# aproposorg/sydr

Hardware: AMD Instinct MI355X
Metric: IQ Msamples/s through 32-ch E/P/L correlators @25 MHz fs (higher is better)
Workload: dtype f64

## Files before the change

### sydr_amd/csrc/correlator_chip.h

```cpp
#pragma once

#include "correlator.h"

#pragma clang fp contract(off)

namespace sdr {

constexpr int kChipMax = 26;
constexpr double kChipMinCodeStep = 1.0 / 25.9;
constexpr double kChipMaxCodeStep = 1.0 / 15.5;
constexpr int kChipRawDwords = 13;
constexpr int kChipRotSlots = 2 * kChipMax + 2;
template <int NT>
constexpr int chip_strip_slots() { return 2 * NT + 1; }

__host__ __device__ __forceinline__ int chip_first_above(double thr, double shift, double inv_step, bool& near) {
    const double u = (thr - shift) * inv_step;
    const double fl = floor(u);
    const double fr = u - fl;
    near = near || fr < kNearInteger || fr > 1.0 - kNearInteger;
    return (int)fl + 1;
}
__host__ __device__ __forceinline__ int chip_first_above_exact(int c, double thr, double step, double shift) {
    auto above = [&](int i) {
        double y = (double)i * step;
        y = y + shift;
        return y > thr;
    };
    if (c >= 1 && above(c - 1)) return (c >= 2 && above(c - 2)) ? c - 2 : c - 1;
    if (c < 0) c = 0;
    if (above(c)) return c;
    return above(c + 1) ? c + 1 : c + 2;
}

template <int B, int E, class F>
__device__ __forceinline__ void static_for(F&& f) {
    if constexpr (B < E) {
        f(std::integral_constant<int, B>{});
        static_for<B + 1, E>(f);
    }
}

__device__ __forceinline__ int wave_min_i32(int x) {
#pragma unroll
    for (int off = 1; off < 64; off <<= 1) {
        const int o = __shfl_xor(x, off, 64);
        x = o < x ? o : x;
    }
    return __builtin_amdgcn_readfirstlane(x);
}

#ifndef SDR_BIASED_CVT
#define SDR_BIASED_CVT 1
#endif
constexpr double kCvtBias = 4224.0;
typedef uint32_t sdr_u32x2 __attribute__((ext_vector_type(2)));
__device__ __forceinline__ double biased_sample(sdr_u32x2& pair, uint32_t w_flipped, uint32_t selector, uint32_t hi_const) {
    pair.y = __builtin_amdgcn_perm(w_flipped, hi_const, selector);
    return __builtin_bit_cast(double, pair);
}
constexpr uint32_t cvt_selector(int byte) { return 0x03020000u | ((uint32_t)(4 + byte) << 8) | 0x0Cu; }

template <int NT>
struct ChipGeom {
    int64_t Tfx, Ufx;
    uint64_t delta[NT];
    int q0, F;
    int head_end, tail_start;
    int m[NT], J[NT];
    int bad;
};

template <int NT, int KM, int KS, int KI>
__host__ __device__ __forceinline__ void chip_geometry(int n, const double* shift, const double* step, const double* inv_step,
                                                       ChipGeom<NT>& g) {
    constexpr int A = NT / 2;
    const double two32 = 4294967296.0;
    g.q0 = (int)ceil(shift[A]);
    double y_last = (double)(n - 1) * step[A];
    y_last = y_last + shift[A];
    const int q_last = (int)ceil(y_last);
    g.F = q_last - g.q0 - 1;
    g.head_end = n, g.tail_start = n;
    if (g.F > 0) {
        bool nr = false;
        g.head_end = chip_first_above_exact(chip_first_above((double)g.q0, shift[A], inv_step[A], nr), (double)g.q0, step[A], shift[A]);
        g.tail_start = chip_first_above_exact(chip_first_above((double)(q_last - 1), shift[A], inv_step[A], nr),
                                              (double)(q_last - 1), step[A], shift[A]);
    }
    g.Tfx = (int64_t)rint(inv_step[A] * two32);
    g.Ufx = (int64_t)floor(-shift[A] * inv_step[A] * two32);
    const int M = (int)(g.Tfx >> 32);
    bool bad = M < 1 || M + 1 > kChipMax || g.F > 16384 || (KM != 0 && M != KM);
#pragma unroll
    for (int t = 0; t < NT; ++t) {
        g.m[t] = M, g.J[t] = 0, g.delta[t] = 0;
        if (t == A) continue;
        const int64_t Ut = (int64_t)floor(-shift[t] * inv_step[t] * two32);
        int j = (int)ceil(shift[t] - shift[A]) - 1;
        int64_t d = (Ut - g.Ufx) + (int64_t)(1 + j) * g.Tfx;
        if (d < 0) {
            d += g.Tfx;
            ++j;
        } else if (d >= g.Tfx) {
            d -= g.Tfx;
            --j;
        }
        bad = bad || d < 0 || d >= g.Tfx;
        g.J[t] = j;
        g.delta[t] = (uint64_t)d;
        g.m[t] = (int)(d >> 32);
        bad = bad || (KS != 0 && (g.m[t] != KS || j != (t < A ? -1 : 0)));
        bad = bad || (KI != 0 && !((j == (t - A) * KI - 1 && g.m[t] == 0) || (j == (t - A) * KI && g.m[t] >= M)));
    }
    g.bad = bad ? 1 : 0;
}

constexpr int kStaticHalf = 13;
constexpr int chip_half(int KM, int KS, int KI) { return KI != 0 ? (KM + 2) / 2 : KS + 1; }
struct ChipRot {
    double urc[kStaticHalf + 1], urs[kStaticHalf + 1];
    double rd0c, rd0s, rd1c, rd1s;
    double biasc[3], biass[3];
};
__host__ __device__ inline void chip_rotations(double dphi, int Dmin, ChipRot& r, int half = kStaticHalf, int cmin = kStaticHalf - 2) {
    double cs[16], sn[16];
    for (int k = 0; k < 16; ++k) sincos_reduced(-(double)k * dphi, &sn[k], &cs[k]);
    for (int k = 1; k <= half; ++k) r.urc[k] = cs[k], r.urs[k] = sn[k];
    r.urc[0] = 1.0, r.urs[0] = 0.0;
    sincos_reduced(-(double)Dmin * dphi, &r.rd0s, &r.rd0c);
    sincos_reduced(-(double)(Dmin + 1) * dphi, &r.rd1s, &r.rd1c);
    for (int st = 1; st < 16; st <<= 1)
        for (int l = 15; l >= st; --l) cs[l] += cs[l - st], sn[l] += sn[l - st];
    for (int i = 0; i < 3; ++i) {
        const int l = cmin + i - 1;
        const double re = cs[l] - sn[l], im = cs[l] + sn[l];
        r.biasc[i] = re * 4224.0, r.biass[i] = im * 4224.0;
    }
}

template <int NT>
struct ChipSetup {
    double dphi;
    double shift[NT], step[NT], inv_step[NT];
    int64_t base;
    ChipGeom<NT> g;
    ChipRot r;
};

template <int NT, int KM, int KS, int KI>
__host__ __device__ inline void chip_setup(int n, int64_t start_sample, int64_t capacity, double carrier_hz, double rem_code,
                                           double code_step, const double* spacing, double fs, int stride, ChipSetup<NT>& S) {
    S = ChipSetup<NT>{};
    S.dphi = carrier_step(carrier_hz, fs);
    const double nd = (double)n;
    for (int t = 0; t < NT; ++t) {
        const double shift = rem_code + spacing[t];
        double stop = code_step * nd;
        stop = stop + shift;
        const double delta = stop - shift;
        S.shift[t] = shift;
        S.step[t] = delta / nd;
        S.inv_step[t] = 1.0 / S.step[t];
    }
    const int64_t base = start_sample % capacity;
    const bool applies = code_step >= kChipMinCodeStep && code_step <= kChipMaxCodeStep && base + n + 32 <= capacity;
    S.base = applies ? base : -1;
    if (applies) {
        chip_geometry<NT, KM, KS, KI>(n, S.shift, S.step, S.inv_step, S.g);
        chip_rotations(S.dphi, (int)(((int64_t)stride * S.g.Tfx) >> 32), S.r, chip_half(KM, KS, KI), KM - chip_half(KM, KS, KI));
    }
}

template <int NT>
struct ChipBlock {
    uint32_t raw[kChipRawDwords];
    int S;
    int dn;
    int ds[NT];
};

template <int NT, bool SINGLE_WAVE, int KM = 0, int KS = 0, int KI = 0>
__device__ __forceinline__ bool correlate_epoch_chip(const void* __restrict__ ring, const void* __restrict__ ring_flipped, int64_t capacity,
                                                     const EpochParams& ep, double dphi, const EpochConsts<NT>& K,
                                                     const ChipGeom<NT>& G, int64_t base, const ChipRot* R,
                                                     const uint32_t* lut, double2* strip_lds, double2* rot, int tid,
                                                     int lane, int stride, int edge_lane, double* accr, double* acci) {
    constexpr int A = NT / 2;
    constexpr int kSlots = chip_strip_slots<NT>();
    const int n = ep.n;
    const double* shift = K.shift;
    const double* step = K.step;
    double2* strip = strip_lds + tid * kSlots;
    const int wlane = threadIdx.x & 63;
#pragma unroll
    for (int t = 0; t < NT; ++t) accr[t] = acci[t] = 0.0;

    const double dphi_u = uniform(dphi), rem_carrier_u = uniform(ep.rem_carrier);
    const int q0 = __builtin_amdgcn_readfirstlane(G.q0);
    const int F = __builtin_amdgcn_readfirstlane(G.F);
    const int head_end = __builtin_amdgcn_readfirstlane(G.head_end);
    const int tail_start = __builtin_amdgcn_readfirstlane(G.tail_start);
    (void)ring_flipped;
    const char* ring_base = static_cast<const char*>(ring) + base * 2;

    static_assert(!(KS != 0 && KI != 0), "either the taps switch inside the block (KS) or with it (KI)");
    constexpr bool kStatic = KM != 0 && (KS != 0 || KI != 0);
    constexpr int kHalf = chip_half(KM, KS, KI);
    double urc[kStatic ? kHalf + 1 : 1], urs[kStatic ? kHalf + 1 : 1];
    double biasc[3] = {0.0, 0.0, 0.0}, biass[3] = {0.0, 0.0, 0.0};
    const double two32 = 4294967296.0;
    int64_t Tfx = G.Tfx;
    int64_t stride_fx = (int64_t)stride * Tfx;
    const int Dmin = (int)(stride_fx >> 32);
    if constexpr (kStatic) asm volatile("" : "+v"(Tfx), "+v"(stride_fx));
    double rd0c = 1.0, rd0s = 0.0, rd1c = 1.0, rd1s = 0.0;
    {
        double sn = 0.0, cs = 0.0;
        if constexpr (kStatic) {
            static_assert(kHalf <= kStaticHalf, "the plan's rotations are laid out for half blocks of up to 13 samples");
#pragma unroll
            for (int k = 1; k <= kHalf; ++k) urc[k] = R->urc[k], urs[k] = R->urs[k];
            rd0c = R->rd0c, rd0s = R->rd0s, rd1c = R->rd1c, rd1s = R->rd1s;
            if constexpr (SDR_BIASED_CVT) {
#pragma unroll
                for (int i = 0; i < 3; ++i) biasc[i] = R->biasc[i], biass[i] = R->biass[i];
            }
        } else {
            if (wlane < kChipMax) {
                sincos_reduced(-(double)wlane * dphi_u, &sn, &cs);
                rot[wlane] = make_double2(cs, sn);
            }
            if constexpr (SDR_BIASED_CVT) {
                double br = (cs - sn) * kCvtBias, bi = (cs + sn) * kCvtBias;
#pragma unroll
                for (int off = 1; off < 32; off <<= 1) {
                    const double o_r = __shfl_up(br, off, 64), o_i = __shfl_up(bi, off, 64);
                    br = wlane >= off ? br + o_r : br;
                    bi = wlane >= off ? bi + o_i : bi;
                }
                double2* const btab = rot + kChipMax;
                if (wlane < kChipMax) btab[wlane + 1] = make_double2(br, bi);
                if (wlane == 0) btab[0] = make_double2(0.0, 0.0);
            }
        }
    }

    bool bad = false;
    const int rounds = F > 0 ? (F + stride - 1) / stride : 0;
    if (rounds > 0) {
        int64_t Ufx = G.Ufx;
        const int M = (int)(G.Tfx >> 32);
        if constexpr (kStatic) asm volatile("" : "+v"(Ufx));
        bad = bad || G.bad != 0;
        int m[NT], J[NT];
        uint64_t delta[NT];
        unsigned evmask = (1u << M) | (2u << M);
#pragma unroll
        for (int t = 0; t < NT; ++t) {
            m[t] = G.m[t], J[t] = G.J[t], delta[t] = G.delta[t];
            if constexpr (kStatic) asm volatile("" : "+v"(m[t]), "+v"(J[t]), "+v"(delta[t]));
            if (t != A) evmask |= (1u << m[t]) | (2u << m[t]);
        }
        const int k_last = M + 1;
        int rank[NT];
#pragma unroll
        for (int t = 0; t < NT; ++t) rank[t] = __builtin_popcount(evmask & ((1u << m[t]) - 1u));
        if constexpr (!kStatic) {
            double sn, cs;
            sincos_reduced(-(double)(Dmin + (wlane & 1)) * dphi_u, &sn, &cs);
            rd0c = lane_value(cs, 0), rd0s = lane_value(sn, 0);
            rd1c = lane_value(cs, 1), rd1s = lane_value(sn, 1);
        }
        asm volatile("" : "+v"(rd0c), "+v"(rd0s), "+v"(rd1c), "+v"(rd1s));
        const uint64_t lane_fx = (uint64_t)((int64_t)lane * Tfx);
        uint64_t u_cur = (uint64_t)(Ufx + (int64_t)q0 * Tfx + (int64_t)two32) + lane_fx;
        const int last_idx = F - 1;

        auto prepare = [&](int round, uint64_t u0, ChipBlock<NT>& b) {
            const int idx = round * stride + lane;
            const bool inside = idx <= last_idx;
            const uint64_t uS = inside ? u0 : (uint64_t)(Ufx + (int64_t)(q0 + last_idx) * Tfx + (int64_t)two32);
            const uint64_t uE = uS + (uint64_t)Tfx;
            int S = (int)(uS >> 32);
            int E = (int)(uE >> 32);
            bool near = (uint32_t)uS + 0x10000u < 0x20000u || (uint32_t)uE + 0x10000u < 0x20000u;
            int split[NT];
#pragma unroll
            for (int t = 0; t < NT; ++t) {
                split[t] = 0;
                if (t == A) continue;
                if constexpr (KI != 0) {
                    split[t] = J[t] == (t - A) * KI ? E - S : 0;
                    continue;
                }
                const uint64_t uT = uS + delta[t];
                near = near || (uint32_t)uT + 0x10000u < 0x20000u;
                split[t] = (int)(uT >> 32) - S;
            }
            if (__builtin_expect(__any(near), 0)) {
                const int q = q0 + 1 + (inside ? idx : last_idx);
                S = chip_first_above_exact(S, (double)(q - 1), step[A], shift[A]);
                E = chip_first_above_exact(E, (double)q, step[A], shift[A]);
#pragma unroll
                for (int t = 0; t < NT; ++t) {
                    if (t == A) continue;
                    const int p0 = q + J[t];
                    const int bt = chip_first_above_exact(S + split[t], (double)p0, step[t], shift[t]);
                    double y = (double)S * step[t];
                    y = y + shift[t];
                    const int at_s = (int)ceil(y);
                    bad = bad || (at_s != p0 && at_s != p0 + 1) || (at_s == p0 + 1 && bt > S);
                    split[t] = bt < S ? 0 : bt - S;
                }
            }
            b.S = S;
            const int nn = E - S;
            b.dn = nn - M;
            bad = bad || (unsigned)b.dn > 1u;
#pragma unroll
            for (int t = 0; t < NT; ++t) {
                b.ds[t] = 0;
                if (t == A) continue;
                const int sp = split[t] > nn ? nn : split[t];
                if constexpr (KI != 0) {
                    bad = bad || !(J[t] == (t - A) * KI ? sp == nn : sp == 0);
                    continue;
                }
                b.ds[t] = sp - m[t];
                bad = bad || (unsigned)b.ds[t] > 1u;
            }
            if constexpr (KS != 0 && NT == 3) bad = bad || b.ds[0] != b.ds[2];
            const char* src = ring_base + (int64_t)S * 2;
            const uint4 w0 = *reinterpret_cast<const uint4*>(src);
            const uint4 w1 = *reinterpret_cast<const uint4*>(src + 16);
            const uint4 w2 = *reinterpret_cast<const uint4*>(src + 32);
            const uint32_t w3 = *reinterpret_cast<const uint32_t*>(src + 48);
            b.raw[0] = w0.x, b.raw[1] = w0.y, b.raw[2] = w0.z, b.raw[3] = w0.w;
            b.raw[4] = w1.x, b.raw[5] = w1.y, b.raw[6] = w1.z, b.raw[7] = w1.w;
            b.raw[8] = w2.x, b.raw[9] = w2.y, b.raw[10] = w2.z, b.raw[11] = w2.w;
            b.raw[12] = w3;
        };

        ChipBlock<NT> blk_a, blk_b;
        prepare(0, u_cur, blk_a);
        double sb, cb;
        sincos_reduced(__builtin_fma(-(double)blk_a.S, dphi_u, rem_carrier_u), &sb, &cb);
        if constexpr (!kStatic) {
            sb = lane <= last_idx ? sb : 0.0;
            cb = lane <= last_idx ? cb : 0.0;
        }
        const int q_lane = q0 + 1 + lane + SDR_LUT_PAD;
        const uint32_t* zero_lq = reinterpret_cast<const uint32_t*>(strip) + 3;
        if constexpr (kStatic) strip[0] = strip[1] = make_double2(0.0, 0.0);

        sdr_u32x2 zI = {0u, 0u}, zQ = {0u, 0u};
        asm volatile("" : "+v"(zI), "+v"(zQ));

        auto process = [&](const ChipBlock<NT>& b, int round, double sbk, double cbk) {
            double pr = 0.0, pi = 0.0;
            double2* wp = strip;
            unsigned evm = evmask;
            int klast = k_last;
            if constexpr (!kStatic) asm volatile("" : "+s"(evm), "+s"(klast));
            constexpr int kAhead = 4;
            double2 rr[kChipMax + kAhead];
            if constexpr (!kStatic) {
#pragma unroll
                for (int k = 0; k < kAhead; ++k) rr[k] = rot[k];
            }
            auto park = [&]() {
                *wp = make_double2(pr, pi);
                ++wp;
                asm volatile("" ::: "memory");
            };
            uint32_t hi_rt = 0x40B00000u;
            uint32_t sel_rt[4] = {cvt_selector(0), cvt_selector(1), cvt_selector(2), cvt_selector(3)};
            if constexpr (!kStatic && SDR_BIASED_CVT) {
                asm volatile("" : "+v"(hi_rt));
                asm volatile("" : "+s"(sel_rt[0]), "+s"(sel_rt[1]), "+s"(sel_rt[2]), "+s"(sel_rt[3]));
            }
            auto sample = [&](auto kc) {
                constexpr int k = decltype(kc)::value;
                double ar, ai;
                if constexpr (SDR_BIASED_CVT) {
                    ar = biased_sample(zI, b.raw[k >> 1], sel_rt[(k & 1) ? 2 : 0], hi_rt);
                    ai = biased_sample(zQ, b.raw[k >> 1], sel_rt[(k & 1) ? 3 : 1], hi_rt);
                } else {
                    const int w = ci8_native((int)b.raw[k >> 1]);
                    ar = (k & 1) ? (double)(int)(int8_t)(w >> 16) : (double)(int)(int8_t)w;
                    ai = (k & 1) ? (double)(w >> 24) : (double)(int)(int8_t)(w >> 8);
                }
                if (k + kAhead < kChipMax) rr[k + kAhead] = rot[k + kAhead];
                const double2 r = rr[k];
                pr = __builtin_fma(-ai, r.y, __builtin_fma(ar, r.x, pr));
                pi = __builtin_fma(ai, r.x, __builtin_fma(ar, r.y, pi));
                if constexpr (SDR_BIASED_CVT) asm volatile("" : "+v"(pr), "+v"(pi), "+v"(zI), "+v"(zQ));
            };
            double capr[3] = {0.0, 0.0, 0.0}, capi[3] = {0.0, 0.0, 0.0};
            if constexpr (kStatic) {
                static_assert(2 * kHalf >= KM + 1 && kHalf < KM, "two halves of at most KS + 1 samples cover the block");
                static_assert(!SDR_BIASED_CVT || (2 * kHalf - KM >= 1 && 2 * kHalf - KM <= 2 && (KS == 0 || KS == kHalf - 1)),
                              "the offset's shares are kept for sums of KM - kHalf, + 1 and + 2 samples: kHalf must be one of the last two");
                uint32_t flipped[kChipRawDwords];
                uint32_t hi_const = 0x40B00000u;
                if constexpr (SDR_BIASED_CVT) {
                    asm volatile("" : "+v"(hi_const));
#pragma unroll
                    for (int i = 0; i < kChipRawDwords; ++i) flipped[i] = b.raw[i];
                }
                static_for<0, KM + 1>([&](auto kc) {
                    constexpr int k = decltype(kc)::value;
                    constexpr int j = k < kHalf ? k : k - kHalf;
                    const int w = ci8_native((int)b.raw[k >> 1]);
                    double ar, ai;
                    if constexpr (SDR_BIASED_CVT) {
                        ar = biased_sample(zI, flipped[k >> 1], cvt_selector((k & 1) ? 2 : 0), hi_const);
                        ai = biased_sample(zQ, flipped[k >> 1], cvt_selector((k & 1) ? 3 : 1), hi_const);
                    } else {
                        ar = (k & 1) ? (double)(int)(int8_t)(w >> 16) : (double)(int)(int8_t)w;
                        ai = (k & 1) ? (double)(w >> 24) : (double)(int)(int8_t)(w >> 8);
                    }
                    if constexpr (KS != 0 && k == KS) capr[0] = pr, capi[0] = pi;
                    if constexpr (k == KM) capr[1] = pr, capi[1] = pi;
                    if constexpr (k == kHalf) capr[2] = pr, capi[2] = pi;
                    if constexpr (j == 0) {
                        pr = ar, pi = ai;
                    } else {
                        pr = __builtin_fma(-ai, urs[j], __builtin_fma(ar, urc[j], pr));
                        pi = __builtin_fma(ai, urc[j], __builtin_fma(ar, urs[j], pi));
                    }
                    if constexpr (SDR_BIASED_CVT) asm volatile("" : "+v"(pr), "+v"(pi), "+v"(zI), "+v"(zQ));
                });
            } else if constexpr (KM != 0) {
                static_for<0, KM>([&](auto kc) {
                    constexpr int k = decltype(kc)::value;
                    if (evm & (1u << k)) park();
                    sample(kc);
                });
                park();
                sample(std::integral_constant<int, KM>{});
                park();
            } else {
#pragma unroll
                for (int k = 0; k <= kChipMax; ++k) {
                    if (evm & (1u << k)) {
                        park();
                        if (k == klast) break;
                    }
                    if (k < kChipMax) {
                        double ar, ai;
                        if constexpr (SDR_BIASED_CVT) {
                            ar = biased_sample(zI, b.raw[k >> 1], sel_rt[(k & 1) ? 2 : 0], hi_rt);
                            ai = biased_sample(zQ, b.raw[k >> 1], sel_rt[(k & 1) ? 3 : 1], hi_rt);
                        } else {
                            const int w = ci8_native((int)b.raw[k >> 1]);
                            ar = (k & 1) ? (double)(int)(int8_t)(w >> 16) : (double)(int)(int8_t)w;
                            ai = (k & 1) ? (double)(w >> 24) : (double)(int)(int8_t)(w >> 8);
                        }
                        if (k + kAhead < kChipMax) rr[k + kAhead] = rot[k + kAhead];
                        const double2 r = rr[k];
                        pr = __builtin_fma(-ai, r.y, __builtin_fma(ar, r.x, pr));
                        pi = __builtin_fma(ai, r.x, __builtin_fma(ar, r.y, pi));
                        if constexpr (SDR_BIASED_CVT) asm volatile("" : "+v"(pr), "+v"(pi), "+v"(zI), "+v"(zQ));
                    }
                }
            }
            double2 ptot;
            if constexpr (kStatic && SDR_BIASED_CVT) {
                constexpr int iFirst = 2 * kHalf - KM;
                pr -= biasc[1], pi -= biass[1];
                capr[1] -= biasc[0], capi[1] -= biass[0];
                capr[2] -= biasc[iFirst], capi[2] -= biass[iFirst];
                if constexpr (KS != 0) capr[0] -= biasc[iFirst - 1], capi[0] -= biass[iFirst - 1];
            }
            if constexpr (kStatic) {
                const double qr = b.dn ? pr : capr[1], qi = b.dn ? pi : capi[1];
                ptot.x = __builtin_fma(-qi, urs[kHalf], __builtin_fma(qr, urc[kHalf], capr[2]));
                ptot.y = __builtin_fma(qi, urc[kHalf], __builtin_fma(qr, urs[kHalf], capi[2]));
            } else {
                ptot = strip[rank[A] + b.dn];
                if constexpr (SDR_BIASED_CVT) {
                    const double2 bb = (rot + kChipMax)[M + b.dn];
                    ptot.x -= bb.x, ptot.y -= bb.y;
                }
            }
            const int first = round * stride;
            const uint32_t* lq;
            if constexpr (kStatic)
                lq = first + lane <= last_idx ? lut + q_lane + first : zero_lq;
            else
                lq = lut + q_lane + (first + lane <= last_idx ? first : last_idx - lane);
            if constexpr (KI != 0) {
                const double xr = __builtin_fma(-sbk, ptot.y, cbk * ptot.x);
                const double xi = __builtin_fma(sbk, ptot.x, cbk * ptot.y);
#pragma unroll
                for (int t = 0; t < NT; ++t) {
                    const double c = __hiloint2double((int)lq[(t - A) * KI], 0);
                    accr[t] = __builtin_fma(c, xr, accr[t]);
                    acci[t] = __builtin_fma(c, xi, acci[t]);
                }
                return;
            }
#pragma unroll
            for (int t = 0; t < NT; ++t) {
                double gr, gi;
                if (t == A) {
                    const double c = __hiloint2double((int)lq[0], 0);
                    gr = c * ptot.x;
                    gi = c * ptot.y;
                } else {
                    double2 ps;
                    if constexpr (kStatic)
                        ps = b.ds[NT == 3 ? 0 : t] ? make_double2(capr[2], capi[2]) : make_double2(capr[0], capi[0]);
                    else {
                        ps = strip[rank[t] + b.ds[t]];
                        if constexpr (SDR_BIASED_CVT) {
                            const double2 bb = (rot + kChipMax)[m[t] + b.ds[t]];
                            ps.x -= bb.x, ps.y -= bb.y;
                        }
                    }
                    const int jt = kStatic ? (t < A ? -1 : 0) : J[t];
                    const double ca = __hiloint2double((int)lq[jt], 0);
                    const double cbn = __hiloint2double((int)lq[jt + 1], 0);
                    const double diff = ca - cbn;
                    gr = __builtin_fma(diff, ps.x, cbn * ptot.x);
                    gi = __builtin_fma(diff, ps.y, cbn * ptot.y);
                }
                accr[t] = __builtin_fma(-sbk, gi, __builtin_fma(cbk, gr, accr[t]));
                acci[t] = __builtin_fma(sbk, gr, __builtin_fma(cbk, gi, acci[t]));
            }
        };

        auto wave_has_work = [&](int round) { return SINGLE_WAVE || round * stride + (lane - wlane) <= last_idx; };
        auto advance = [&](const ChipBlock<NT>& from, const ChipBlock<NT>& to, int to_round) {
            const unsigned dd = (unsigned)(to.S - from.S - Dmin);
            const bool alive = to_round * stride + lane <= last_idx;
            bad = bad || (alive && dd > 1u);
            const double rc_ = dd ? rd1c : rd0c, rs_ = dd ? rd1s : rd0s;
            const double cbn = __builtin_fma(cb, rc_, -sb * rs_);
            const double sbn = __builtin_fma(sb, rc_, cb * rs_);
            if constexpr (kStatic) {
                cb = cbn, sb = sbn;
            } else {
                cb = alive ? cbn : 0.0;
                sb = alive ? sbn : 0.0;
            }
        };

        for (int it = 0; it < rounds / 2; ++it) {
            const double sb0 = sb, cb0 = cb;
            u_cur += (uint64_t)stride_fx;
            prepare(2 * it + 1, u_cur, blk_b);
            advance(blk_a, blk_b, 2 * it + 1);
            if (wave_has_work(2 * it)) process(blk_a, 2 * it, sb0, cb0);
            const double sb1 = sb, cb1 = cb;
            if (2 * it + 2 < rounds) {
                u_cur += (uint64_t)stride_fx;
                prepare(2 * it + 2, u_cur, blk_a);
                advance(blk_b, blk_a, 2 * it + 2);
            }
            if (wave_has_work(2 * it + 1)) process(blk_b, 2 * it + 1, sb1, cb1);
        }
        if ((rounds & 1) && wave_has_work(rounds - 1)) process(blk_a, rounds - 1, sb, cb);
    }

    if (__any(bad)) return false;
    if (edge_lane >= 0) {
        if (head_end + (n - tail_start) > 64) {
            for (int off = 0; off < head_end + (n - tail_start); off += 64)
                edge_samples<SDR_FMT_CI8, NT>(ring, capacity, ep, dphi, shift, step, lut, edge_lane + off, head_end, tail_start, accr, acci, base);
        } else {
            edge_samples<SDR_FMT_CI8, NT>(ring, capacity, ep, dphi, shift, step, lut, edge_lane, head_end, tail_start, accr, acci, base);
        }
    }
    return true;
}

__device__ __forceinline__ bool chip_variant_applies(const EpochParams& ep, int64_t capacity) {
    return ep.code_step >= kChipMinCodeStep && ep.code_step <= kChipMaxCodeStep &&
           ep.start_sample % capacity + ep.n + 32 <= capacity;
}

}
```

Baseline: 95470.

## Walk chip block boundaries with 32-bit carry flags instead of per-block exact search

For static-tap single-wave variants, the per-block start sample and tap-split flags now come from a 32-bit fixed-point fraction walk, where carries decide whether a boundary shifts. The exact floating-point boundary search runs only when some lane's fraction is near an integer. The flags are recomputed inside process from the stored fraction rather than carried in registers. The loop is split into unclamped main rounds and clamped tail rounds, and alternating zero-pair registers are used for odd and even samples in the biased conversion. The aim is to cut integer and FP work in block preparation and relieve dependency chains, at the cost of more code and extra register constraints.

```diff
diff --git a/sydr_amd/csrc/correlator_chip.h b/sydr_amd/csrc/correlator_chip.h
--- a/sydr_amd/csrc/correlator_chip.h
+++ b/sydr_amd/csrc/correlator_chip.h
@@ -54,6 +54,9 @@
 #define SDR_BIASED_CVT 1
 #endif
 constexpr double kCvtBias = 4224.0;
+#ifndef SDR_ALT_PAIRS
+#define SDR_ALT_PAIRS 1
+#endif
 typedef uint32_t sdr_u32x2 __attribute__((ext_vector_type(2)));
 __device__ __forceinline__ double biased_sample(sdr_u32x2& pair, uint32_t w_flipped, uint32_t selector, uint32_t hi_const) {
     pair.y = __builtin_amdgcn_perm(w_flipped, hi_const, selector);
@@ -172,12 +175,45 @@
     }
 }
 
+struct ChipWalk {
+    int S;
+    uint32_t f;
+};
+__host__ __device__ __forceinline__ ChipWalk chip_walk_at(uint64_t u) { return ChipWalk{(int)(u >> 32), (uint32_t)u}; }
+__host__ __device__ __forceinline__ bool chip_carry(uint32_t a, uint32_t b, uint32_t& sum) { return __builtin_add_overflow(a, b, &sum); }
+__host__ __device__ __forceinline__ bool chip_near_sample(uint32_t fr) { return fr + 0x10000u < 0x20000u; }
+__host__ __device__ __forceinline__ bool chip_walk_step(ChipWalk& w, uint32_t stride_lo, int Dmin) {
+    const bool dd = chip_carry(w.f, stride_lo, w.f);
+    w.S = w.S + Dmin + (dd ? 1 : 0);
+    return dd;
+}
+__host__ __device__ __forceinline__ ChipWalk chip_walk_clamp(const ChipWalk& w, bool inside, const ChipWalk& w_last) {
+    return ChipWalk{inside ? w.S : w_last.S, inside ? w.f : w_last.f};
+}
+template <int NT, int KI>
+__host__ __device__ __forceinline__ void chip_walk_flags(uint32_t f, uint32_t T_lo, const uint32_t* delta_lo, bool& dn, bool* ds, bool& near) {
+    uint32_t fE;
+    dn = chip_carry(f, T_lo, fE);
+    near = chip_near_sample(f) || chip_near_sample(fE);
+#pragma unroll
+    for (int t = 0; t < NT; ++t) {
+        ds[t] = false;
+        if (t == NT / 2 || KI != 0) continue;
+        uint32_t fT;
+        ds[t] = chip_carry(f, delta_lo[t], fT);
+        near = near || chip_near_sample(fT);
+    }
+}
+
 template <int NT>
 struct ChipBlock {
     uint32_t raw[kChipRawDwords];
     int S;
     int dn;
     int ds[NT];
+    uint32_t f;
+    int slow;
+    int adj;
 };
 
 template <int NT, bool SINGLE_WAVE, int KM = 0, int KS = 0, int KI = 0>
@@ -206,6 +242,7 @@
 
     static_assert(!(KS != 0 && KI != 0), "either the taps switch inside the block (KS) or with it (KI)");
     constexpr bool kStatic = KM != 0 && (KS != 0 || KI != 0);
+    constexpr bool kWalk = kStatic && (KS != 0 || NT > 3);
     constexpr int kHalf = chip_half(KM, KS, KI);
     double urc[kStatic ? kHalf + 1 : 1], urs[kStatic ? kHalf + 1 : 1];
     double biasc[3] = {0.0, 0.0, 0.0}, biass[3] = {0.0, 0.0, 0.0};
@@ -224,7 +261,10 @@
             rd0c = R->rd0c, rd0s = R->rd0s, rd1c = R->rd1c, rd1s = R->rd1s;
             if constexpr (SDR_BIASED_CVT) {
 #pragma unroll
-                for (int i = 0; i < 3; ++i) biasc[i] = R->biasc[i], biass[i] = R->biass[i];
+                for (int i = 0; i < 3; ++i) {
+                    biasc[i] = R->biasc[i], biass[i] = R->biass[i];
+                    if constexpr (kWalk && (kHalf >= 12 || NT > 3)) asm volatile("" : "+v"(biasc[i]), "+v"(biass[i]));
+                }
             }
         } else {
             if (wlane < kChipMax) {
@@ -342,8 +382,100 @@
             b.raw[12] = w3;
         };
 
+        const uint32_t T_lo = (uint32_t)Tfx, stride_lo = (uint32_t)stride_fx;
+        uint32_t delta_lo[NT];
+#pragma unroll
+        for (int t = 0; t < NT; ++t) delta_lo[t] = (uint32_t)delta[t];
+        int bad_v = 0;
+        int Dmin_v = Dmin;
+        if constexpr (kWalk) asm volatile("" : "+v"(bad_v), "+v"(Dmin_v));
+        auto prepare_walk = [&](auto clampc, int round, const ChipWalk& w_in, ChipBlock<NT>& b) {
+            constexpr bool kClamp = decltype(clampc)::value;
+            const int idx = round * stride + lane;
+            bool inside = true;
+            ChipWalk w = w_in;
+            if constexpr (kClamp) {
+                inside = idx <= last_idx;
+                w = chip_walk_clamp(w_in, inside, chip_walk_at((uint64_t)(Ufx + (int64_t)(q0 + last_idx) * Tfx + (int64_t)two32)));
+            }
+            bool dn, ds[NT], near;
+            chip_walk_flags<NT, KI>(w.f, T_lo, delta_lo, dn, ds, near);
+            if constexpr (KS != 0 && NT == 3) near = near || ds[0] != ds[2];
+            b.f = w.f;
+            b.slow = 0;
+            uint32_t off;
+            if (__builtin_expect(__any(near), 0)) {
+                int S = w.S;
+                int E = S + M + (dn ? 1 : 0);
+                int split[NT];
+#pragma unroll
+                for (int t = 0; t < NT; ++t) {
+                    split[t] = 0;
+                    if (t == A) continue;
+                    if constexpr (KI != 0)
+                        split[t] = J[t] == (t - A) * KI ? E - S : 0;
+                    else
+                        split[t] = m[t] + (ds[t] ? 1 : 0);
+                }
+                bool wrong = false;
+                const int q = q0 + 1 + (inside ? idx : last_idx);
+                S = chip_first_above_exact(S, (double)(q - 1), step[A], shift[A]);
+                E = chip_first_above_exact(E, (double)q, step[A], shift[A]);
+#pragma unroll
+                for (int t = 0; t < NT; ++t) {
+                    if (t == A) continue;
+                    const int p0 = q + J[t];
+                    const int bt = chip_first_above_exact(S + split[t], (double)p0, step[t], shift[t]);
+                    double y = (double)S * step[t];
+                    y = y + shift[t];
+                    const int at_s = (int)ceil(y);
+                    wrong = wrong || (at_s != p0 && at_s != p0 + 1) || (at_s == p0 + 1 && bt > S);
+                    split[t] = bt < S ? 0 : bt - S;
+                }
+                const int nn = E - S;
+                b.dn = nn - M;
+                wrong = wrong || (unsigned)b.dn > 1u;
+#pragma unroll
+                for (int t = 0; t < NT; ++t) {
+                    b.ds[t] = 0;
+                    if (t == A) continue;
+                    const int sp = split[t] > nn ? nn : split[t];
+                    if constexpr (KI != 0) {
+                        wrong = wrong || !(J[t] == (t - A) * KI ? sp == nn : sp == 0);
+                        continue;
+                    }
+                    b.ds[t] = sp - m[t];
+                    wrong = wrong || (unsigned)b.ds[t] > 1u;
+                }
+                if constexpr (KS != 0 && NT == 3) wrong = wrong || b.ds[0] != b.ds[2];
+                bad_v |= wrong ? 1 : 0;
+                b.adj = S - w.S;
+                b.slow = 1;
+                off = (uint32_t)S << 1;
+            } else {
+                off = (uint32_t)w.S << 1;
+            }
+            asm volatile("" : "+s"(b.slow));
+            const char* src = ring_base + off;
+            const uint4 w0 = *reinterpret_cast<const uint4*>(src);
+            const uint4 w1 = *reinterpret_cast<const uint4*>(src + 16);
+            const uint4 w2 = *reinterpret_cast<const uint4*>(src + 32);
+            const uint32_t w3 = *reinterpret_cast<const uint32_t*>(src + 48);
+            b.raw[0] = w0.x, b.raw[1] = w0.y, b.raw[2] = w0.z, b.raw[3] = w0.w;
+            b.raw[4] = w1.x, b.raw[5] = w1.y, b.raw[6] = w1.z, b.raw[7] = w1.w;
+            b.raw[8] = w2.x, b.raw[9] = w2.y, b.raw[10] = w2.z, b.raw[11] = w2.w;
+            b.raw[12] = w3;
+        };
+
         ChipBlock<NT> blk_a, blk_b;
-        prepare(0, u_cur, blk_a);
+        ChipWalk walk = chip_walk_at(u_cur);
+        if constexpr (kWalk) {
+            prepare_walk(std::true_type{}, 0, walk, blk_a);
+            const ChipWalk w0 = chip_walk_clamp(walk, lane <= last_idx, chip_walk_at((uint64_t)(Ufx + (int64_t)(q0 + last_idx) * Tfx + (int64_t)two32)));
+            blk_a.S = w0.S + (blk_a.slow ? blk_a.adj : 0);
+        } else {
+            prepare(0, u_cur, blk_a);
+        }
         double sb, cb;
         sincos_reduced(__builtin_fma(-(double)blk_a.S, dphi_u, rem_carrier_u), &sb, &cb);
         if constexpr (!kStatic) {
@@ -356,8 +488,13 @@
 
         sdr_u32x2 zI = {0u, 0u}, zQ = {0u, 0u};
         asm volatile("" : "+v"(zI), "+v"(zQ));
-
-        auto process = [&](const ChipBlock<NT>& b, int round, double sbk, double cbk) {
+        sdr_u32x2 zI2 = {0u, 0u}, zQ2 = {0u, 0u};
+        if constexpr (kWalk) asm volatile("" : "+v"(zI2), "+v"(zQ2));
+
+        uint32_t hi_epoch = 0x40B00000u;
+        if constexpr (kWalk && SDR_BIASED_CVT) asm volatile("" : "+v"(hi_epoch));
+        auto process = [&](const ChipBlock<NT>& b, int round, double sbk, double cbk, auto clampc) {
+            constexpr bool kClamp = decltype(clampc)::value;
             double pr = 0.0, pi = 0.0;
             double2* wp = strip;
             unsigned evm = evmask;
@@ -403,9 +540,9 @@
                 static_assert(!SDR_BIASED_CVT || (2 * kHalf - KM >= 1 && 2 * kHalf - KM <= 2 && (KS == 0 || KS == kHalf - 1)),
                               "the offset's shares are kept for sums of KM - kHalf, + 1 and + 2 samples: kHalf must be one of the last two");
                 uint32_t flipped[kChipRawDwords];
-                uint32_t hi_const = 0x40B00000u;
+                uint32_t hi_const = hi_epoch;
                 if constexpr (SDR_BIASED_CVT) {
-                    asm volatile("" : "+v"(hi_const));
+                    if constexpr (!kWalk) asm volatile("" : "+v"(hi_const));
 #pragma unroll
                     for (int i = 0; i < kChipRawDwords; ++i) flipped[i] = b.raw[i];
                 }
@@ -415,8 +552,8 @@
                     const int w = ci8_native((int)b.raw[k >> 1]);
                     double ar, ai;
                     if constexpr (SDR_BIASED_CVT) {
-                        ar = biased_sample(zI, flipped[k >> 1], cvt_selector((k & 1) ? 2 : 0), hi_const);
-                        ai = biased_sample(zQ, flipped[k >> 1], cvt_selector((k & 1) ? 3 : 1), hi_const);
+                        ar = biased_sample(kWalk && SDR_ALT_PAIRS && (k & 1) ? zI2 : zI, flipped[k >> 1], cvt_selector((k & 1) ? 2 : 0), hi_const);
+                        ai = biased_sample(kWalk && SDR_ALT_PAIRS && (k & 1) ? zQ2 : zQ, flipped[k >> 1], cvt_selector((k & 1) ? 3 : 1), hi_const);
                     } else {
                         ar = (k & 1) ? (double)(int)(int8_t)(w >> 16) : (double)(int)(int8_t)w;
                         ai = (k & 1) ? (double)(w >> 24) : (double)(int)(int8_t)(w >> 8);
@@ -430,7 +567,10 @@
                         pr = __builtin_fma(-ai, urs[j], __builtin_fma(ar, urc[j], pr));
                         pi = __builtin_fma(ai, urc[j], __builtin_fma(ar, urs[j], pi));
                     }
-                    if constexpr (SDR_BIASED_CVT) asm volatile("" : "+v"(pr), "+v"(pi), "+v"(zI), "+v"(zQ));
+                    if constexpr (SDR_BIASED_CVT) {
+                        if constexpr (kWalk && SDR_ALT_PAIRS && (k & 1)) asm volatile("" : "+v"(pr), "+v"(pi), "+v"(zI2), "+v"(zQ2));
+                        else asm volatile("" : "+v"(pr), "+v"(pi), "+v"(zI), "+v"(zQ));
+                    }
                 });
             } else if constexpr (KM != 0) {
                 static_for<0, KM>([&](auto kc) {
@@ -474,8 +614,25 @@
                 capr[2] -= biasc[iFirst], capi[2] -= biass[iFirst];
                 if constexpr (KS != 0) capr[0] -= biasc[iFirst - 1], capi[0] -= biass[iFirst - 1];
             }
+            bool dnf = false, dsf[NT];
+#pragma unroll
+            for (int t = 0; t < NT; ++t) dsf[t] = false;
+            if constexpr (kWalk) {
+                if (__builtin_expect(b.slow != 0, 0)) {
+                    dnf = b.dn != 0;
+#pragma unroll
+                    for (int t = 0; t < NT; ++t) dsf[t] = b.ds[t] != 0;
+                    asm volatile("" : "+v"(pr), "+v"(pi));
+                } else {
+                    uint32_t f = b.f;
+                    asm volatile("" : "+v"(f), "+v"(pr), "+v"(pi));
+                    bool nr;
+                    chip_walk_flags<NT, KI>(f, T_lo, delta_lo, dnf, dsf, nr);
+                }
+            }
             if constexpr (kStatic) {
-                const double qr = b.dn ? pr : capr[1], qi = b.dn ? pi : capi[1];
+                if constexpr (!kWalk) dnf = b.dn != 0;
+                const double qr = dnf ? pr : capr[1], qi = dnf ? pi : capi[1];
                 ptot.x = __builtin_fma(-qi, urs[kHalf], __builtin_fma(qr, urc[kHalf], capr[2]));
                 ptot.y = __builtin_fma(qi, urc[kHalf], __builtin_fma(qr, urs[kHalf], capi[2]));
             } else {
@@ -488,7 +645,7 @@
             const int first = round * stride;
             const uint32_t* lq;
             if constexpr (kStatic)
-                lq = first + lane <= last_idx ? lut + q_lane + first : zero_lq;
+                lq = !kClamp || first + lane <= last_idx ? lut + q_lane + first : zero_lq;
             else
                 lq = lut + q_lane + (first + lane <= last_idx ? first : last_idx - lane);
             if constexpr (KI != 0) {
@@ -512,7 +669,7 @@
                 } else {
                     double2 ps;
                     if constexpr (kStatic)
-                        ps = b.ds[NT == 3 ? 0 : t] ? make_double2(capr[2], capi[2]) : make_double2(capr[0], capi[0]);
+                        ps = (kWalk ? dsf[NT == 3 ? 0 : t] : b.ds[NT == 3 ? 0 : t] != 0) ? make_double2(capr[2], capi[2]) : make_double2(capr[0], capi[0]);
                     else {
                         ps = strip[rank[t] + b.ds[t]];
                         if constexpr (SDR_BIASED_CVT) {
@@ -548,21 +705,68 @@
             }
         };
 
-        for (int it = 0; it < rounds / 2; ++it) {
-            const double sb0 = sb, cb0 = cb;
-            u_cur += (uint64_t)stride_fx;
-            prepare(2 * it + 1, u_cur, blk_b);
-            advance(blk_a, blk_b, 2 * it + 1);
-            if (wave_has_work(2 * it)) process(blk_a, 2 * it, sb0, cb0);
-            const double sb1 = sb, cb1 = cb;
-            if (2 * it + 2 < rounds) {
+        static_assert(SINGLE_WAVE || !kWalk, "the straight-line forms give a wave an epoch of its own");
+        if constexpr (kWalk) {
+            auto next_block = [&](auto clampc, const ChipBlock<NT>& from, ChipBlock<NT>& to, int to_round) {
+                constexpr bool kClamp = decltype(clampc)::value;
+                bool dd = chip_walk_step(walk, stride_lo, Dmin_v);
+                prepare_walk(clampc, to_round, walk, to);
+                if (__builtin_expect((from.slow | to.slow) != 0, 0)) {
+                    bool alive = true;
+                    int d = dd ? 1 : 0;
+                    if constexpr (kClamp) {
+                        alive = to_round * stride + lane <= last_idx;
+                        const int S_last = (int)((uint64_t)(Ufx + (int64_t)(q0 + last_idx) * Tfx + (int64_t)two32) >> 32);
+                        d = alive ? d : S_last - (walk.S - d - Dmin_v) - Dmin_v;
+                    }
+                    if (to.slow) d += to.adj;
+                    if (from.slow) d -= from.adj;
+                    bad_v |= alive && (unsigned)d > 1u ? 1 : 0;
+                    dd = d != 0;
+                    asm volatile("");
+                }
+                const double rc_ = dd ? rd1c : rd0c, rs_ = dd ? rd1s : rd0s;
+                const double cbn = __builtin_fma(cb, rc_, -sb * rs_);
+                const double sbn = __builtin_fma(sb, rc_, cb * rs_);
+                cb = cbn, sb = sbn;
+                asm volatile("" : "+v"(cb), "+v"(sb));
+            };
+            auto settle = [&]() {
+#pragma unroll
+                for (int t = 0; t < NT; ++t) asm volatile("" : "+v"(accr[t]), "+v"(acci[t]));
+            };
+            auto round_pair = [&](auto clampc, int it) {
+                const double sb0 = sb, cb0 = cb;
+                next_block(clampc, blk_a, blk_b, 2 * it + 1);
+                process(blk_a, 2 * it, sb0, cb0, clampc);
+                settle();
+                const double sb1 = sb, cb1 = cb;
+                if (!decltype(clampc)::value || 2 * it + 2 < rounds) next_block(clampc, blk_b, blk_a, 2 * it + 2);
+                process(blk_b, 2 * it + 1, sb1, cb1, clampc);
+                settle();
+            };
+            const int plain = rounds >= 2 ? (rounds - 2) / 2 : 0;
+            for (int it = 0; it < plain; ++it) round_pair(std::false_type{}, it);
+            for (int it = plain; it < rounds / 2; ++it) round_pair(std::true_type{}, it);
+            if (rounds & 1) process(blk_a, rounds - 1, sb, cb, std::true_type{});
+        } else {
+            for (int it = 0; it < rounds / 2; ++it) {
+                const double sb0 = sb, cb0 = cb;
                 u_cur += (uint64_t)stride_fx;
-                prepare(2 * it + 2, u_cur, blk_a);
-                advance(blk_b, blk_a, 2 * it + 2);
-            }
-            if (wave_has_work(2 * it + 1)) process(blk_b, 2 * it + 1, sb1, cb1);
+                prepare(2 * it + 1, u_cur, blk_b);
+                advance(blk_a, blk_b, 2 * it + 1);
+                if (wave_has_work(2 * it)) process(blk_a, 2 * it, sb0, cb0, std::true_type{});
+                const double sb1 = sb, cb1 = cb;
+                if (2 * it + 2 < rounds) {
+                    u_cur += (uint64_t)stride_fx;
+                    prepare(2 * it + 2, u_cur, blk_a);
+                    advance(blk_b, blk_a, 2 * it + 2);
+                }
+                if (wave_has_work(2 * it + 1)) process(blk_b, 2 * it + 1, sb1, cb1, std::true_type{});
+            }
+            if ((rounds & 1) && wave_has_work(rounds - 1)) process(blk_a, rounds - 1, sb, cb, std::true_type{});
         }
-        if ((rounds & 1) && wave_has_work(rounds - 1)) process(blk_a, rounds - 1, sb, cb);
+        bad = bad || bad_v != 0;
     }
 
     if (__any(bad)) return false;
```

New measurement: 99290 (median of 6 runs). 1.04x the previous value.
